# ishine/Prior-DiffuSE

Measured on AMD Instinct MI355X. Metric: enhanced-audio sec/sec (RTF), 6-step fast sampling, B=32, higher is better.
Workload: dtype f16x2; 1 GPU; B=32 x 4 s 16 kHz utterances per GPU, [B,2,401,161] spectrograms, GCRN prior + DiffUNet1 6-step sampling, STFT..ISTFT, seeded random weights; global_batch=32, frames=401, parallelism=batch-shard x1, graph=True, streams_per_gpu=1, batches_in_flight=3

## Files before the change

### include/pdse.h

```cpp
#ifndef PDSE_H
#define PDSE_H
#include <stdint.h>

#ifdef __cplusplus
extern "C" {
#endif

#define PDSE_ABI_VERSION 9

typedef void* pdse_stream_t;

enum pdse_act { PDSE_ACT_NONE = 0, PDSE_ACT_PRELU = 1, PDSE_ACT_ELU = 2, PDSE_ACT_SIGMOID = 3 };

enum pdse_epi {
  PDSE_EPI_LINEAR = 0,
  PDSE_EPI_GLU = 1,
  PDSE_EPI_BIGLU = 2
};

typedef struct pdse_src {
  const float* ptr;
  int64_t sb, sc, st, sf;
  int32_t C;
  int32_t act;
// ... 409 lines not shown
  int64_t bias_sb;
  const float* blc;
  const float* brc;
  const float* bc2;
  float slope;
  int32_t C2;
  float* out;
  int64_t out_sb, out_sc, out_st, out_sf, out_off;
  int32_t hp_par, nx_n;
  uint16_t* nx_hp;
  int64_t nx_hp_sb;
  int32_t nx_Tp, nx_Fp, nx_t0, nx_f0;
  int32_t nx_row0;
  int32_t nx_par;
  const float* nx_add;
  int64_t add_sb, add_sc, add_st, add_sf;
  float* nx_out[2];
  int64_t nx_sb[2], nx_sc[2], nx_st[2], nx_sf[2];
  const float* nx_bias[3];
  int64_t nx_bias_sb[3];
  int32_t skip_Fh;
  int32_t nx_items;
  int32_t qexp[4];
} pdse_bglu_desc;

typedef struct pdse_planes_desc {
  const float* in;
  int64_t in_sb, in_sc, in_st, in_sf;
  uint16_t* hp;
  int64_t hp_sb;
  int32_t hp_Tp, hp_Fp, hp_t0, hp_f0;
  int32_t B, T, F, np;
  const float* in1;
  const float* w[2];
  const float* bias[2];
  int64_t bias_sb;
  uint16_t* hp1;
  int32_t cin0, cin1, nd, pad_;
} pdse_planes_desc;

#define PDSE_METRICS_SSNR 0
#define PDSE_METRICS_LLR 1
#define PDSE_METRICS_WSS 2
#define PDSE_METRICS_FWSNRSEG 3
#define PDSE_METRICS_OFF_WIN 0
#define PDSE_METRICS_OFF_BASIS 512
// ... 157 lines not shown
```

### prior-diffuse_amd/_lib.py

```python
import contextlib
import ctypes as C
import os

_HERE = os.path.dirname(os.path.abspath(__file__))
LIB_PATH = os.environ.get("PDSE_LIB") or os.path.join(_HERE, "libpdse.so")

ABI_VERSION = 9

ACT_NONE, ACT_PRELU, ACT_ELU, ACT_SIGMOID = 0, 1, 2, 3
EPI_LINEAR, EPI_GLU, EPI_BIGLU = 0, 1, 2
EW_DIV, EW_UPDATE, EW_UPDATE_FINAL, EW_COPY, EW_ADD_MUL = 0, 1, 2, 3, 4
(OP_GCONV, OP_TIME, OP_EW, OP_COMPAND, OP_WAVPREP, OP_OLA, OP_SIGMA, OP_LN, OP_LSTM,
 OP_ROWLN, OP_CHLN, OP_ATTN, OP_GRU, OP_GNCOMB, OP_AHAM, OP_QSAMPLE, OP_TRANSPOSE, OP_TCM, OP_CRM, OP_GCRNLAST,
 OP_MASKLOSS, OP_GLSTM, OP_TCM2, OP_BGLU, OP_PLANES, OP_GLSTMP, OP_TCM2S, OP_DENSE, OP_ROWLNB, OP_METRICS, OP_RESAMPLE, OP_RANGE) = range(32)
MASKLOSS_BLOCKS = 32

_fp = C.c_void_p
_i32, _i64, _f32 = C.c_int32, C.c_int64, C.c_float


class Src(C.Structure):
    _fields_ = [("ptr", _fp), ("sb", _i64), ("sc", _i64), ("st", _i64), ("sf", _i64),
                ("C", _i32), ("act", _i32), ("blk", _i32), ("pad_", _i32)]

# ... 155 lines not shown


TCM2S_MAX = 20


class Tcm2sDesc(C.Structure):
    _fields_ = [("blk", Tcm2Desc * TCM2S_MAX), ("flags", _fp), ("status", _fp), ("n", _i32), ("pad_", _i32)]


class BgluDesc(C.Structure):
    _fields_ = [("hp", _fp), ("hp_sb", _i64), ("hp_Tp", _i32), ("hp_Fp", _i32), ("hp_t0", _i32), ("hp_f0", _i32),
                ("x0", Src), ("x1", Src), ("Tin", _i32), ("Fin", _i32), ("ntaps", _i32), ("sf_in", _i32),
                ("tap_dt", _i32 * 10), ("tap_df", _i32 * 10), ("p1mask", _i32), ("Fout1", _i32),
                ("B", _i32), ("Tout", _i32), ("Fout", _i32), ("np", _i32),
                ("w0", _fp), ("w1", _fp), ("w2", _fp), ("w3", _fp), ("wlc", _fp), ("wrc", _fp), ("wc2", _fp), ("wc2v", _fp),
                ("nx_w", _fp), ("bias0", _fp), ("bias1", _fp), ("bias0_t0", _fp), ("bias1_t0", _fp), ("bias_sb", _i64),
                ("blc", _fp), ("brc", _fp), ("bc2", _fp), ("slope", _f32), ("C2", _i32),
                ("out", _fp), ("out_sb", _i64), ("out_sc", _i64), ("out_st", _i64), ("out_sf", _i64), ("out_off", _i64),
                ("hp_par", _i32), ("nx_n", _i32),
                ("nx_hp", _fp), ("nx_hp_sb", _i64), ("nx_Tp", _i32), ("nx_Fp", _i32), ("nx_t0", _i32), ("nx_f0", _i32),
                ("nx_row0", _i32), ("nx_par", _i32),
                ("nx_add", _fp), ("add_sb", _i64), ("add_sc", _i64), ("add_st", _i64), ("add_sf", _i64),
                ("nx_out", _fp * 2), ("nx_sb", _i64 * 2), ("nx_sc", _i64 * 2), ("nx_st", _i64 * 2), ("nx_sf", _i64 * 2),
                ("nx_bias", _fp * 3), ("nx_bias_sb", _i64 * 3), ("skip_Fh", _i32), ("nx_items", _i32), ("qexp", _i32 * 4)]


class PlanesDesc(C.Structure):
    _fields_ = [("in_", _fp), ("in_sb", _i64), ("in_sc", _i64), ("in_st", _i64), ("in_sf", _i64),
                ("hp", _fp), ("hp_sb", _i64), ("hp_Tp", _i32), ("hp_Fp", _i32), ("hp_t0", _i32), ("hp_f0", _i32),
                ("B", _i32), ("T", _i32), ("F", _i32), ("np", _i32),
                ("in1", _fp), ("w", _fp * 2), ("bias", _fp * 2), ("bias_sb", _i64), ("hp1", _fp),
                ("cin0", _i32), ("cin1", _i32), ("nd", _i32), ("pad_", _i32)]


class CrmDesc(C.Structure):
    _fields_ = [("x", _fp), ("o", _fp), ("ri", _fp), ("out", _fp), ("a1", _f32), ("b1", _f32), ("a2", _f32), ("b2", _f32),
                ("a3", _f32), ("b3", _f32), ("plane", _i32), ("B", _i32), ("mode", _i32), ("pad_", _i32)]


class GcrnLastDesc(C.Structure):
    _fields_ = [("in0", _fp), ("in1", _fp), ("w1", _fp), ("w2", _fp), ("fcT", _fp), ("fcb", _fp), ("out", _fp),
                ("out_sb", _i64), ("b1", _f32), ("b2", _f32), ("bn_scale", _f32), ("bn_shift", _f32), ("B", _i32), ("T", _i32),
                ("fcp", _fp)]


class MetricsDesc(C.Structure):
    _fields_ = [("clean", _fp), ("proc", _fp), ("lens_host", _fp), ("lens", _fp), ("tables", _fp), ("frames", _fp),
# ... 238 lines not shown
```

### prior-diffuse_amd/csrc/bglu.hip

```cpp
#include <hip/hip_runtime.h>
#include <stdint.h>
#include <stdio.h>
#include <stdlib.h>

#include "pdse.h"
#include "pdse_internal.h"

#include "gconv_common.h"

#ifndef BGLU_ST_AUX
#define BGLU_ST_AUX 0
#endif

namespace {

#ifdef BGLU_DIAG
__device__ unsigned long long g_bglu_slots[97];
#endif

constexpr int popc(int m) { return m ? (m & 1) + popc(m >> 1) : 0; }
constexpr int rank_of(int m, int tap) { return popc(m & ((1 << tap) - 1)); }

__device__ __forceinline__ void glds16(const void* g, void* l) {
  __builtin_amdgcn_global_load_lds((const __attribute__((address_space(1))) void*)g, (__attribute__((address_space(3))) void*)l,
// ... 92 lines not shown

__device__ __forceinline__ float vmax(const float a, const float b) {
  float r;
  asm("v_max_f32 %0, %1, %2" : "=v"(r) : "v"(a), "v"(b));
  return r;
}

#define BGLU_FLOATS 512
enum { F_BL = 0, F_BR = 32, F_BL0 = 64, F_BR0 = 96, F_BLC = 128, F_BRC = 160, F_BC2 = 192, F_NXB = 256, F_WC2V = 352 };

template <int NT, int P1MASK, int C2, int NXN, bool IN4, int NP>
struct bglu_cfg {
  static constexpr int WV = 8;
  static constexpr int NB = IN4 ? 3 : 2 * NT;
  static constexpr int NT1 = popc(P1MASK), NB1 = 2 * NT1;
  static constexpr bool DUAL = P1MASK != 0;
  static constexpr int BS = NP * 64;
  static constexpr int o_gL = 0, o_gR = NB * BS, o_gL1 = 2 * NB * BS, o_gR1 = o_gL1 + NB1 * BS, o_lc = o_gR1 + NB1 * BS,
                       o_rc = o_lc + 2 * BS, o_c2 = o_rc + 2 * BS, o_nx = o_c2 + (C2 == 64 ? 4 * BS : 0),
                       o_f = o_nx + NXN * 4 * BS;
  static constexpr size_t lds_bytes = (size_t)o_f * sizeof(uint4) + BGLU_FLOATS * sizeof(float);
};

template <int NT, int P1MASK, int C2, int NXN, bool IN4, int NP>
__global__ __launch_bounds__(512, 2) void bglu_kernel(const pdse_bglu_desc d) {
  using CF = bglu_cfg<NT, P1MASK, C2, NXN, IN4, NP>;
  constexpr int WV = CF::WV, NB = CF::NB, NB1 = CF::NB1, BS = CF::BS;
  constexpr bool DUAL = CF::DUAL;
  extern __shared__ uint4 img[];
  const int tid = threadIdx.x;
  const int lane = tid & 63, wave = tid >> 6;
  const int col = lane & 31, h = lane >> 5;
  const int b = blockIdx.y;
  const int P = d.Tout * d.Fout;
  constexpr int PE = NP == 2 ? PDSE_F16_ACT_EXP : 0;
  const int qG = NP == 2 ? d.qexp[0] : 0, qLC = NP == 2 ? d.qexp[1] : 0, qC2 = NP == 2 ? d.qexp[2] : 0, qNX = NP == 2 ? d.qexp[3] : 0;
  [[maybe_unused]] const float s_in = pow2i(PE), s_G = pow2i(-qG), s_LC = pow2i(-(PE + qLC)), s_C2 = pow2i(-qC2), s_NX = pow2i(-qNX),
                               s_C2out = pow2i(-(PE + qC2)), s_NXout = pow2i(-(PE + qNX)), s_NXin = pow2i(PE + qNX);

  {
    const uint4* const srcs[8] = {reinterpret_cast<const uint4*>(d.w0), reinterpret_cast<const uint4*>(d.w1),
                                  reinterpret_cast<const uint4*>(d.w2), reinterpret_cast<const uint4*>(d.w3),
                                  reinterpret_cast<const uint4*>(d.wlc), reinterpret_cast<const uint4*>(d.wrc),
                                  reinterpret_cast<const uint4*>(d.wc2), reinterpret_cast<const uint4*>(d.nx_w)};
    const int cnt[8] = {NB * NP, NB * NP, NB1 * NP, NB1 * NP, 2 * NP, 2 * NP, C2 == 64 ? 4 * NP : 0, NXN * 4 * NP};
    constexpr int total = CF::o_f >> 6;
    for (int c = __builtin_amdgcn_readfirstlane(wave); c < total; c += WV) {
      int cc = c;
// ... 499 lines not shown
      bv[s_][i] = src[(int64_t)(2 * i + h) * d.in_sc];
    }
  };
  request(0, 0);
  for (int k0 = 0; k0 < K; k0 += 64) {
    if (k0 + 32 < K) request(k0 + 32, 1);
#pragma unroll
    for (int i = 0; i < 16; ++i) acc = __builtin_amdgcn_mfma_f32_32x32x2f32(av[0][i], bv[0][i], acc, 0, 0, 0);
    if (k0 + 32 >= K) break;
    if (k0 + 64 < K) request(k0 + 64, 0);
#pragma unroll
    for (int i = 0; i < 16; ++i) acc = __builtin_amdgcn_mfma_f32_32x32x2f32(av[1][i], bv[1][i], acc, 0, 0, 0);
  }
  if (!live) return;
  uint4 p[2][NP];
  split16p<NP>(acc, p, NP == 2 ? pow2i(PDSE_F16_ACT_EXP) : 1.0f);
  uint4* const base = reinterpret_cast<uint4*>((di ? d.hp1 : d.hp) + (int64_t)b * d.hp_sb) + ((int64_t)(t + d.hp_t0) * 4 + h) * (NP * d.hp_Fp) + f + d.hp_f0;
#pragma unroll
  for (int q = 0; q < 2; ++q)
#pragma unroll
    for (int pl = 0; pl < NP; ++pl) base[(2 * q * NP + pl) * d.hp_Fp] = p[q][pl];
}

template <int NT, int P1MASK, int C2, int NXN, bool IN4, int NP>
int launch(const pdse_bglu_desc* d, hipStream_t s) {
  using CF = bglu_cfg<NT, P1MASK, C2, NXN, IN4, NP>;
  const int P = d->Tout * d->Fout;
  const int rounds = (((P + 31) >> 5) + CF::WV - 1) / CF::WV;
  static const int wgs = PDSE_DIAG_ENV("PDSE_BGLU_WGS") ? atoi(PDSE_DIAG_ENV("PDSE_BGLU_WGS")) : 256;
  int gx = (wgs + d->B - 1) / d->B;
  if (gx > rounds) gx = rounds;
  if (gx < 1) gx = 1;
  if (CF::lds_bytes > 160 * 1024) {
    pdse_set_error("bglu: LDS image too large");
    return 1;
  }
  const void* fn = (const void*)bglu_kernel<NT, P1MASK, C2, NXN, IN4, NP>;
  static unsigned long long attr_mask = 0;
  if (pdse_lds_attr(fn, &attr_mask, "bglu lds attribute")) return 1;
#ifdef BGLU_DIAG
  static unsigned long long zs[97];
  for (int k = 0; k < 97; ++k) zs[k] = 0;
  (void)hipMemcpyToSymbol(HIP_SYMBOL(g_bglu_slots), zs, sizeof(zs));
#endif
  hipLaunchKernelGGL((bglu_kernel<NT, P1MASK, C2, NXN, IN4, NP>), dim3(gx, d->B, 1), dim3(64 * CF::WV), CF::lds_bytes, s, *d);
#ifdef BGLU_DIAG
  (void)hipStreamSynchronize(s);
  (void)hipMemcpyFromSymbol(zs, HIP_SYMBOL(g_bglu_slots), sizeof(zs));
  if (zs[96]) {
    fprintf(stderr, "bglu slots NT %d P1 %d C2 %d NXN %d NP %d (cycles per slot and tile, %llu tiles):", NT, P1MASK, C2, NXN, NP, zs[96]);
    double tot = 0;
    for (int k = 0; k < 96; ++k)
      if (zs[k]) {
        fprintf(stderr, " %d:%.0f", k, (double)zs[k] / (double)zs[96]);
        tot += (double)zs[k] / (double)zs[96];
      }
    fprintf(stderr, " | sum %.0f\n", tot);
  }
#endif
  return pdse_check_launch("bglu");
}

template <int NP>
int dispatch(const pdse_bglu_desc* d, hipStream_t s) {
  if (d->x0.ptr) {
    if (d->nx_n == 3) return launch<10, 0, 64, 3, true, NP>(d, s);
  } else if (d->p1mask) {
    if (d->ntaps == 4 && d->p1mask == 5 && d->C2 == 64 && d->nx_n == 1) return launch<4, 5, 64, 1, false, NP>(d, s);
    if (d->ntaps == 6 && d->p1mask == 27 && d->C2 == 1 && d->nx_n == 0) return launch<6, 27, 1, 0, false, NP>(d, s);
  } else {
    if (d->ntaps == 6 && d->C2 == 64 && d->nx_n == 3) return launch<6, 0, 64, 3, false, NP>(d, s);
    if (d->ntaps == 6 && d->C2 == 64 && d->nx_n == 0) return launch<6, 0, 64, 0, false, NP>(d, s);
  }
  pdse_set_error("bglu: no instantiation for this (taps, phases, C2, chained tiles)");
  return 1;
}

}

int pdse_bglu_launch(const pdse_bglu_desc* d, hipStream_t s) {
  if (!d || !d->w0 || !d->w1 || !d->wlc || !d->wrc || !d->bias0 || !d->bias1 || !d->blc || !d->brc || !d->bc2) {
    pdse_set_error("bglu: null operand");
    return 1;
  }
  if (!(d->slope <= 1.0f)) {
    pdse_set_error("bglu: PReLU slope must be <= 1 (max form); use the korder 2 kernels otherwise");
    return 1;
  }
  if (d->B < 1 || d->Tout < 1 || d->Fout < 1 || !(d->np == 3 || d->np == 2 || d->np == 1) || !(d->C2 == 64 || d->C2 == 1) || d->nx_n < 0 ||
      d->nx_n > 3 || d->ntaps < 1 || d->ntaps > 10) {
    pdse_set_error("bglu: bad geometry (np in {1, 2, 3}, C2 in {64, 1}, nx_n <= 3, ntaps <= 10)");
    return 1;
  }
  if (d->p1mask && d->Fout1 > d->Fout) {
    pdse_set_error("bglu: Fout1 > Fout");
    return 1;
  }
  if ((d->C2 == 64 && !d->wc2) || (d->C2 == 1 && (!d->wc2v || !d->out)) || (d->C2 == 64 && d->nx_n == 0 && !d->out) || (d->nx_n > 0 && (!d->nx_w || !d->nx_hp)) ||
      (d->nx_n > 1 && !d->nx_out[0]) || (d->nx_n > 2 && !d->nx_out[1]) || (d->p1mask && (!d->w2 || !d->w3))) {
    pdse_set_error("bglu: an operand of the selected form is missing");
    return 1;
  }
  if (!d->x0.ptr) {
// ... 44 lines not shown
      return ((sb | sc | st | sf) & 3) == 0 && (reinterpret_cast<uintptr_t>(p) & 15) == 0;
    };
    if (d->nx_add && !c4_ok(d->nx_add, d->add_sb, d->add_sc, d->add_st, d->add_sf)) {
      pdse_set_error("bglu: the addend is kept in groups of four channels: strides in multiples of 4 floats, 16-byte aligned base");
      return 1;
    }
    for (int i = 0; i + 1 < d->nx_n; ++i) {
      if ((long long)(d->B + 1) * d->nx_sb[i] * 4 >= (1ll << 32)) {
        pdse_set_error("bglu: skip tensor exceeds 32-bit lane offsets");
        return 1;
      }
      if (!c4_ok(d->nx_out[i], d->nx_sb[i], d->nx_sc[i], d->nx_st[i], d->nx_sf[i])) {
        pdse_set_error("bglu: skip tensors are kept in groups of four channels: strides in multiples of 4 floats, 16-byte aligned base");
        return 1;
      }
    }
  }
  if (d->np == 2) {
    for (int i = 0; i < 4; ++i)
      if (d->qexp[i] < -40 || d->qexp[i] > 40) {
        pdse_set_error("bglu: qexp (f16x2 weight exponents) out of range");
        return 1;
      }
    return dispatch<2>(d, s);
  }
  return d->np == 3 ? dispatch<3>(d, s) : dispatch<1>(d, s);
}

int pdse_bglu_set_form(int form) {
  static int cur = -1;
  if (form < -1 || form > 0) return -2;
  const int prev = cur;
  cur = form;
  return prev;
}

int pdse_planes_launch(const pdse_planes_desc* d, hipStream_t s) {
  if (!d || !d->in || !d->hp || d->B < 1 || d->T < 1 || d->F < 1 || !(d->np == 3 || d->np == 2 || d->np == 1)) {
    pdse_set_error("planes: bad argument");
    return 1;
  }
  if (d->hp_t0 < 0 || d->hp_f0 < 0 || d->hp_t0 + d->T > d->hp_Tp || d->hp_f0 + d->F > d->hp_Fp) {
    pdse_set_error("planes: the tensor does not fit hp");
    return 1;
  }
  if (d->w[0]) {
    if (d->nd < 1 || d->nd > 2 || d->cin0 < 32 || d->cin1 < 0 || (d->cin0 & 31) || (d->cin1 & 31) || d->cin0 + d->cin1 > 128 || (d->cin1 > 0 && !d->in1) || (d->nd == 2 && (!d->w[1] || !d->hp1)) ||
        d->B > 65535) {
      pdse_set_error("planes: the convolution form takes 1 or 2 weight sets, up to 128 input channels (multiples of 32) over one or two sources");
// ... 20 lines not shown
```

### prior-diffuse_amd/csrc/capi.hip

```cpp
#include <hip/hip_runtime.h>
#include <stdint.h>
#include <stdio.h>
#include <string.h>

#include <new>
#include <string>
#include <vector>

#include "pdse.h"
#include "pdse_internal.h"

static thread_local std::string g_err;

void pdse_set_error(const char* msg) { g_err = msg ? msg : "unknown error"; }

int pdse_check_hip(hipError_t e, const char* what) {
  if (e == hipSuccess) return 0;
  g_err = std::string(what) + ": " + hipGetErrorString(e);
  return 1;
}

int pdse_check_launch(const char* what) { return pdse_check_hip(hipGetLastError(), what); }

int pdse_lds_attr(const void* fn, unsigned long long* mask, const char* what) {
// ... 55 lines not shown

static int op_size(int kind) {
  switch (kind) {
#define X(KIND, stem, entry) case PDSE_OP_##KIND: return (int)sizeof(pdse_##stem##_desc);
    PDSE_OPS(X)
#undef X
    default: return -1;
  }
}

static int launch_op(const pdse_op& op, hipStream_t s) {
  switch (op.kind) {
#define X(KIND, stem, entry) case PDSE_OP_##KIND: return pdse_##stem##_launch(&op.d.stem, s);
    PDSE_OPS(X)
#undef X
    default: pdse_set_error("plan: unknown op kind"); return 1;
  }
}

static bool names_odd_phase(const pdse_op& op) {
  return op.kind == PDSE_OP_GCONV && op.d.gconv.korder == 5 && op.d.gconv.p1mask != 0 && op.d.gconv.w2 == nullptr;
}

static int check_follows(const pdse_plan* p, const pdse_op& op) {
  if (p->ops.empty() || !names_odd_phase(p->ops.back())) return 0;
  if (op.kind != PDSE_OP_GCONV) {
    pdse_set_error("plan: the operator behind a gconv that names its odd phase (p1mask, korder 5) must be that phase");
    return 1;
  }
  return pdse_gconv_pair_check(&p->ops.back().d.gconv, &op.d.gconv);
}

static int launch_at(const pdse_plan* p, const int i, const int end, hipStream_t s, int* n) {
  const pdse_op& op = p->ops[i];
  *n = 1;
  if (names_odd_phase(op) && i + 1 < end) {
    *n = 2;
    return pdse_gconv4_pair_launch(&op.d.gconv, &p->ops[i + 1].d.gconv, s);
  }
  return launch_op(op, s);
}

template <typename D>
static int validate_desc(const D*) { return 0; }
static int validate_desc(const pdse_range_desc* d) { return pdse_range_validate(d); }

extern "C" {

int pdse_abi_version(void) { return PDSE_ABI_VERSION; }
const char* pdse_last_error(void) { return g_err.c_str(); }
int pdse_desc_size(int op_kind) { return op_size(op_kind); }

#define X(KIND, stem, entry) \
  int entry(const pdse_##stem##_desc* d, pdse_stream_t s) { return validate_desc(d) ? 1 : pdse_##stem##_launch(d, (hipStream_t)s); }
PDSE_OPS(X)
#undef X

int pdse_plan_create(pdse_plan** out) {
  if (!out) {
    pdse_set_error("plan_create: null out");
    return 1;
// ... 391 lines not shown
```

### prior-diffuse_amd/csrc/pdse_internal.h

```cpp
#ifndef PDSE_INTERNAL_H
#define PDSE_INTERNAL_H
#include <hip/hip_runtime.h>

#include "pdse.h"

void pdse_set_error(const char* msg);
int pdse_check_launch(const char* what);
int pdse_check_hip(hipError_t e, const char* what);
int pdse_lds_attr(const void* fn, unsigned long long* mask, const char* what);
#ifdef PDSE_DIAG
#define PDSE_DIAG_ENV(name) (getenv(name))
#else
#define PDSE_DIAG_ENV(name) ((const char*)nullptr)
#endif

#define PDSE_OPS(X)                                                                            \
  X(GCONV, gconv, pdse_gconv_f32)                                                              \
  X(TIME, time, pdse_time_embed_f32)                                                           \
  X(EW, ew, pdse_ew_f32)                                                                       \
  X(COMPAND, compand, pdse_compand_f32)                                                        \
  X(WAVPREP, wavprep, pdse_wavprep_f32)                                                        \
  X(OLA, ola, pdse_ola_f32)                                                                    \
  X(SIGMA, sigma, pdse_sigma_mask_f32)                                                         \
  X(LN, ln, pdse_layernorm_f32)                                                                \
// ... 11 lines not shown
  X(GCRNLAST, gcrnlast, pdse_gcrnlast_f32)                                                     \
  X(MASKLOSS, maskloss, pdse_masked_mse_f32)                                                   \
  X(GLSTM, glstm, pdse_glstm_f32)                                                              \
  X(TCM2, tcm2, pdse_tcm2_bf16x3)                                                              \
  X(BGLU, bglu, pdse_bglu_planes)                                                              \
  X(PLANES, planes, pdse_split_planes)                                                         \
  X(GLSTMP, glstmp, pdse_glstm_persistent_f32)                             \
  X(TCM2S, tcm2s, pdse_tcm2_stack_bf16x3)    \
  X(DENSE, dense, pdse_dense_layer_bf16x3)                                 \
  X(ROWLNB, rowlnb, pdse_rowln_blocked_f32)                                                    \
  X(METRICS, metrics, pdse_quality_metrics_f32)                          \
  X(RESAMPLE, resample, pdse_pcm_resample_f32)                          \
  X(RANGE, range, pdse_range_hist)

#define X(KIND, stem, entry) int pdse_##stem##_launch(const pdse_##stem##_desc* d, hipStream_t s);
PDSE_OPS(X)
#undef X
int pdse_gconv2_launch(const pdse_gconv_desc* d, hipStream_t s);
int pdse_gconv3_launch(const pdse_gconv_desc* d, hipStream_t s);
int pdse_gconv4_launch(const pdse_gconv_desc* d, hipStream_t s);
int pdse_gconv_pair_check(const pdse_gconv_desc* d, const pdse_gconv_desc* e);
int pdse_gconv4_pair_check(const pdse_gconv_desc* d, const pdse_gconv_desc* e);
int pdse_gconv4_pair_launch(const pdse_gconv_desc* d, const pdse_gconv_desc* e, hipStream_t s);
int pdse_stoi_launch(const pdse_metrics_desc* d, hipStream_t s);
int pdse_gru3_launch(const pdse_gru_desc* d, hipStream_t s);
int pdse_range_validate(const pdse_range_desc* d);
#endif
```

### prior-diffuse_amd/nets.py

```python
import ctypes as C

import numpy as np
import torch

from . import _lib as L
from . import packing as P

F0 = 161
BIG = 1 << 30

TAG_NONE, TAG_EPS_BLOCK, TAG_EPS_CONV1, TAG_TCM, TAG_PRIOR, TAG_LSTM, TAG_SIGNAL, TAG_EW = range(8)


class WeightBank:

    def __init__(self):
        self.items = {}
        self.keep = []
        self.owners = []

    def token(self, obj):
        if obj is None:
            return None
        for i, o in enumerate(self.owners):
# ... 226 lines not shown


def nc8(C_, T, F):
    return C_ * T * F, T * F * 8, F * 8, 8


def nc8_out(C_, T, F):
    return C_ * T * F, T * F * 8, 1, F * 8, 8


class EpsNetPlan(PlanBase):

    ENC_F = [161, 79, 39, 19, 9, 4]
    fused_tcm = True
    chain_conv1 = True
    compose_stage1 = True
    split_bf16 = True
    split_tcm = True
    plane_h = True
    tcm_stack = True
    parity_planes = True
    planes = 2
    TCM_F16 = True
    NSLOT = 20

    def __init__(self, ctx, sd, B, T, time_cond=True, nsteps=1, plan=None, table=None, with_pre=None, split_bf16=None,
                 planes=None, plane_h=None, exclusive=False, frames=None):
        with_pre = time_cond if with_pre is None else with_pre
        if split_bf16 is not None:
            self.split_bf16 = bool(split_bf16)
        if planes is not None:
            if int(planes) not in (1, 2, 3):
                raise ValueError("planes is 3 (bf16x3), 2 (f16x2) or 1 (bf16 mode)")
            self.planes = int(planes)
        if plane_h is not None:
            self.plane_h = bool(plane_h)
        if self.planes == 1:
            self.plane_h = True
        self.tcm_planes = 3 if (self.planes == 2 and not self.TCM_F16) else self.planes
        self.use_tcm_stack = bool(self.tcm_stack and exclusive)
        self.frames = frames
        if frames is not None and (self.force_generic or not self.fused_tcm):
            raise ValueError("exact ragged batches need a fused TCM form (csrc/tcm.hip, csrc/tcm2.hip): the three-launch form has no frames table")
        self.sd = sd
        ok = (self.split_bf16 and self.chain_conv1 and self.compose_stage1 and time_cond and with_pre and not self.force_generic
              and all(float(P._np(sd[k])[0]) <= 1.0 for k in sd if k.endswith(".weight") and P._np(sd[k]).shape == (1,)))
        if not ok:
            if self.planes == 1:
                raise ValueError("bf16 mode needs the chained split-bf16 DiffUNet1 path (PReLU slopes <= 1)")
            self.plane_h = False
            if self.planes == 2:
                self.planes = self.tcm_planes = 3
        super().__init__(ctx, plan, ns=(ctx.bank.token(sd), bool(time_cond), bool(with_pre), self.fused_tcm, self.chain_conv1,
                                        self.compose_stage1, self.split_bf16, self.split_tcm,
                                        ctx.bank.token(table), str(self.plane_h), self.planes, self.parity_planes))
        self.sd, self.B, self.T, self.time_cond, self.nsteps = sd, B, T, time_cond, nsteps
        self.with_pre = with_pre
        a = ctx.alloc
        self.x = a(B, 2, T, F0)
        self.x_init = a(B, 2, T, F0) if self.with_pre else None
        self.out = a(B, 2, T, F0)
        self.H = a(B, 32, T + 1, F0)
        self.H2 = a(B, 32, T + 1, F0)
        self.Pskip = [[None] + [a(B + 1, 32, T, self.ENC_F[k]) for k in range(1, 5)] for _ in range(2)]
        self.zero32 = self.upw("zero32", lambda: np.zeros(32))
        self.en = [a(B, 64, T, f) for f in self.ENC_F[1:5]] + [a(B, 64, 4, T)]
        self.tcm_a, self.tcm_b = a(B, 256, T), a(B, 256, T)
        self.tcm_h, self.tcm_g = a(B, 64, T), a(B, 64, T)
        self.tcm_hs = [ctx.alloc_u16(*P.tcm2_hs_shape(B, T, self.tcm_planes)) for _ in range(2)]
        self._tcm_stack = None
        self.tcm_flags = torch.zeros(B * ((T + 31) // 32), dtype=torch.int32, device=ctx.device)
        self.tcm_status = torch.zeros(4, dtype=torch.int32, device=ctx.device)
        ctx.keep += [self.tcm_flags, self.tcm_status]
        self.dec = [a(B, 64, T, 79), a(B, 64, T, 79)]
        if self.plane_h:
            self.hp_en = {k: ctx.alloc_u16(*P.hp_shape(B + 1, T, self.ENC_F[k - 1], self.planes)) for k in range(2, 6)}
            self.hp_de = {k: ctx.alloc_u16(*P.hp_shape(B + 1, T, self.ENC_F[k], self.planes)) for k in range(1, 6)}
            self.hp_de5b = ctx.alloc_u16(*P.hp_shape(B + 1, T, self.ENC_F[5], self.planes))
            for k, t_ in self.hp_en.items():
                self.named("hp_en%d" % k, t_)
            for k, t_ in self.hp_de.items():
                self.named("hp_de%d" % k, t_)
            self.named("hp_de5b", self.hp_de5b)
        for name, t_ in (("x", self.x), ("x_init", self.x_init), ("en5", self.en[4]), ("tcm_a", self.tcm_a), ("tcm_b", self.tcm_b),
                         ("tcm_hs0", self.tcm_hs[0]), ("tcm_hs1", self.tcm_hs[1])):
            if t_ is not None:
                self.named(name, t_)
        if time_cond:
            self.tsteps = a(nsteps, B, zero=True)
            self.tbias = a(nsteps, B, self.NSLOT * 32)
            self.temb = a(nsteps, B, 512)
            self._prep_time(table)

    def w(self, k):
        return P._np(self.sd[k])

    def _stage_fold(self):
        st = []
        for k in range(1, 6):
            W1 = self.w("en.conv%d.conv1.weight" % k)[:, :, 0, 0]
# ... 240 lines not shown

    def _residual_split(self, p, dil, xin, xout, hin, hout, p_next, mode=0):
        npl = self.tcm_planes
        d = L.Tcm2Desc()
        self.apply(d, self.fields("%s.split%d.np%d" % (p if mode == 0 else p_next, mode, npl),
                                  lambda: P.tcm2_fields(self.sd, p, p_next, npl, mode)))
        d.x = xin.data_ptr()
        if mode == 0:
            d.x_out, d.hs = xout.data_ptr(), hin.data_ptr()
        if p_next is not None:
            d.hs_out = hout.data_ptr()
        d.dil, d.B, d.T, d.mode, d.np = dil, self.B, self.T, mode, npl
        d.frames = Ctx.ptr(self.frames)
        if mode == 0 and self._tcm_stack is not None:
            self._tcm_stack.append(d)
        else:
            self.add(d, TAG_TCM)

    def _plane_stage(self, kind):
        return self.plane_h is True

    def _bglu(self, label, make, *, hp=None, F_in=None, x0=None, x1=None, taps, sf_in, Fout, p1mask=0, Fout1=0, slope, C2,
              bias, out=None, out_strides=None, out_off=0, nx_hp=None, nx_F=None, nx_row0=False, nx_add=None,
              nx_out=(), nx_bias=(), hp_par=False, nx_par=False, skip_F=0):
        B, T, npl = self.B, self.T, self.planes
        d = L.BgluDesc()
        self.apply(d, self.fields("bglu:%s:%d" % (label, npl), make))
        if hp is not None:
            shp = P.hp_shape(B + 1, T, F_in, npl)
            d.hp, d.hp_sb, d.hp_Tp, d.hp_Fp, d.hp_t0, d.hp_f0 = hp.data_ptr(), int(np.prod(shp[1:])), shp[1], shp[4], P.HP_T0, P.HP_F0
            d.hp_par = 1 if hp_par else 0
        else:
            d.x0, d.x1 = x0, x1
        d.Tin, d.Fin = T, (F_in if F_in is not None else F0)
        d.ntaps, d.sf_in = len(taps), sf_in
        for i, (dt_, df_) in enumerate(taps):
            d.tap_dt[i], d.tap_df[i] = int(dt_), int(df_)
        d.p1mask, d.Fout1 = p1mask, Fout1
        d.B, d.Tout, d.Fout, d.np = B, T, Fout, npl
        tb, o0, o1, o0t, o1t, sb = bias
        if tb is not None:
            d.bias0, d.bias1, d.bias_sb = Ctx.ptr(tb, o0), Ctx.ptr(tb, o1), sb
            if o0t is not None:
                d.bias0_t0, d.bias1_t0 = Ctx.ptr(tb, o0t), Ctx.ptr(tb, o1t)
        d.slope, d.C2 = float(slope), C2
        if out is not None:
            d.out = Ctx.ptr(out)
            d.out_sb, d.out_sc, d.out_st, d.out_sf = out_strides
            d.out_off = out_off
        d.skip_Fh = (skip_F + 1) // 2 if (skip_F and self.parity_planes) else 0
        d.nx_n = (1 if nx_hp is not None else 0) + len(nx_out)
        d.nx_items = B + 1
        assert all(t_.shape[0] == B + 1 for t_, *_ in nx_out) and (nx_hp is None or nx_hp.shape[0] == B + 1)
        if nx_hp is not None:
            shp = P.hp_shape(B + 1, T, nx_F, npl)
            d.nx_hp, d.nx_hp_sb, d.nx_Tp, d.nx_Fp, d.nx_t0, d.nx_f0 = (nx_hp.data_ptr(), int(np.prod(shp[1:])), shp[1], shp[4],
                                                                      P.HP_T0, P.HP_F0)
            d.nx_row0 = 1 if nx_row0 else 0
            d.nx_par = 1 if nx_par else 0
        if nx_add is not None:
            t_, sb_, sc_, st_, sf_ = nx_add
            d.nx_add, d.add_sb, d.add_sc, d.add_st, d.add_sf = Ctx.ptr(t_), sb_, sc_, st_, sf_
        for i, (t_, sb_, sc_, st_, sf_) in enumerate(nx_out):
            d.nx_out[i] = Ctx.ptr(t_)
            d.nx_sb[i], d.nx_sc[i], d.nx_st[i], d.nx_sf[i] = sb_, sc_, st_, sf_
        for i, (t_, off_, sb_) in enumerate(nx_bias):
            d.nx_bias[i], d.nx_bias_sb[i] = Ctx.ptr(t_, off_), sb_
        self.add(d, TAG_EPS_BLOCK)
        return d

    def _encoder_planes(self, step, x, x_init):
        B, T, npl = self.B, self.T, self.planes
        sbb = self.NSLOT * 32
        tb = self.tbias

        def slot(sl):
            return self._bias_for(step, sl)[1]

        for k in range(1, 6):
            p = "en.conv%d" % k
            Fin, Fo = self.ENC_F[k - 1], self.ENC_F[k]
            kw = 5 if k == 1 else 3
            kk, taps = P.conv_taps(2, kw, 1)
            chained = k < 5
            pn = "en.conv%d" % (k + 1)

            def nx_weights(k=k, pn=pn):
                if k == 5:
                    return []
                ws = [self.w(pn + ".conv1.weight")[:, :, 0, 0]]
# ... 16 lines not shown
            kwargs = dict(taps=taps, sf_in=2, Fout=Fo, slope=self._slope("en.en%d.1.weight" % k), C2=64, **src)
            if chained:
                sk = [(self.Pskip[di][k], 32 * T * Fo, 4 * T * Fo, 4 * Fo, 4) for di in range(2)]
                kwargs.update(nx_hp=self.hp_en[k + 1], nx_F=Fo, nx_row0=True, nx_out=sk, nx_par=self.parity_planes, skip_F=Fo,
                              nx_bias=[(tb, slot(k), sbb)] + [(tb, slot(5 + 5 * di + (5 - k)), sbb) for di in range(2)])
            else:
                kwargs.update(out=self.en[4], out_strides=(64 * 4 * T, 4 * T, 1, T))
            self._bglu("en%d" % k, make, bias=bias or (None, 0, 0, None, None, 0), **kwargs)

    def _decoders_planes(self, step, tcm_out, out):
        B, T, npl = self.B, self.T, self.planes
        pd = L.PlanesDesc()
        pd.in_, pd.in1 = tcm_out.data_ptr(), self.en[4].data_ptr()
        pd.in_sb, pd.in_sc, pd.in_st, pd.in_sf = 256 * T, 4 * T, 1, T
        shp = P.hp_shape(B + 1, T, 4, npl)
        pd.hp, pd.hp1 = self.hp_de[5].data_ptr(), self.hp_de5b.data_ptr()
        pd.hp_sb, pd.hp_Tp, pd.hp_Fp, pd.hp_t0, pd.hp_f0 = int(np.prod(shp[1:])), shp[1], shp[4], P.HP_T0, P.HP_F0
        pd.B, pd.T, pd.F, pd.np, pd.cin0, pd.cin1, pd.nd = B, T, 4, npl, 64, 64, 2
        for di, de in enumerate(("de_real", "de_imag")):
            tb, off, sbb = self._bias_for(step, 5 + 5 * di)
            pd.w[di] = self.upw("%s.de5.0.conv1.kmajor" % de, lambda de=de: self.w("%s.de5.0.conv1.weight" % de)[:, :, 0, 0]).data_ptr()
            pd.bias[di], pd.bias_sb = Ctx.ptr(tb, off), sbb
        self.add(pd, TAG_EPS_CONV1)
        for di, de in enumerate(("de_real", "de_imag")):
            for n, k in enumerate((5, 4, 3, 2, 1)):
                p = "%s.de%d.0" % (de, k)
                Fin = self.ENC_F[k]
                kw = 5 if k == 1 else 3
                Fo = 2 * (Fin - 1) + kw
                kk0, taps0 = P.convT_phase_taps(2, kw, 0)
                kk1, taps1 = P.convT_phase_taps(2, kw, 1)
                mask = sum(1 << taps0.index(tp) for tp in taps1)
                C2 = 64 if k > 1 else 1
                bn = "%s.de%d.2" % (de, k) if k > 1 else None

                def make(p=p, k=k, de=de, kk0=kk0, kk1=kk1, C2=C2, bn=bn):
                    g = dict(w0=P.convT_kmat(self.sd[p + ".l.weight"], kk0), w1=P.convT_kmat(self.sd[p + ".r.weight"], kk0),
                             w2=P.convT_kmat(self.sd[p + ".l.weight"], kk1), w3=P.convT_kmat(self.sd[p + ".r.weight"], kk1))
                    nxw = [self.w("%s.de%d.0.conv1.weight" % (de, k - 1))[:, :, 0, 0].T[:, :64]] if k > 1 else []
                    return P.bglu_fields(self.sd, p, True, C2, bn, g, nxw, npl, True)

                kwargs = dict(hp=self.hp_de5b if (k == 5 and di == 1) else self.hp_de[k], F_in=Fin, taps=taps0, sf_in=1, Fout=(Fo + 1) // 2, p1mask=mask, Fout1=Fo // 2,
                              slope=self._slope("%s.de%d.3.weight" % (de, k)) if k > 1 else 1.0, C2=C2,
                              bias=(None, 0, 0, None, None, 0))
                if k > 1:
                    kwargs.update(nx_hp=self.hp_de[k - 1], nx_F=Fo, nx_add=(self.Pskip[di][k - 1], 32 * T * Fo, 4 * T * Fo, 4 * Fo, 4), skip_F=Fo,
                                  nx_bias=[(self.zero32, 0, 0)])
                else:
                    kwargs.update(out=out, out_strides=(2 * T * F0, T * F0, F0, 2), out_off=di * T * F0)
                self._bglu(p, make, **kwargs)

    def build_step(self, step=0, x=None, x_init=None, out=None):
        B, T = self.B, self.T
        x = self.x if x is None else x
        out = self.out if out is None else out
        x_init = self.x_init if x_init is None else x_init
        key = (x.data_ptr(), 0 if x_init is None else x_init.data_ptr(), out.data_ptr())
        tmpl = getattr(self, "_tmpl", None)
        if tmpl is not None and tmpl[0] == key and self.time_cond:
            _, step0, items = tmpl
            lo = self.tbias.data_ptr()
            hi = lo + self.tbias.numel() * 4
            delta = (step - step0) * B * self.NSLOT * 32 * 4
            for d, tag in items:
                d2 = type(d).from_buffer_copy(d)
                if isinstance(d2, L.GconvDesc):
                    for f in ("bias0", "bias1", "bias0_t0", "bias1_t0", "padrow"):
                        v = getattr(d2, f)
                        if v and lo <= v < hi:
                            setattr(d2, f, v + delta)
                    for i in range(d2.nx_n):
                        v = d2.nx_bias[i]
                        if v and lo <= v < hi:
# ... 806 lines not shown
```

Baseline: 10010 audio_s/s.

## Pair real and imaginary decoder BGLU blocks into one launch per stage

Reorders the decoder so each stage's real and imaginary BGLU blocks sit next to each other, and runs the two twins as a single kernel launch. blockIdx.z selects which twin's descriptor a block uses. The decoder plane buffers are doubled so each twin gets its own slice, and a validation step checks the twins share geometry and do not overlap in memory. This removes five launches per step and fills the GPU with twice as many workgroups for the small decoder stages, at the cost of a larger kernel argument block and more plane memory.

```diff
diff --git a/include/pdse.h b/include/pdse.h
--- a/include/pdse.h
+++ b/include/pdse.h
@@ -455,6 +455,7 @@
   int32_t skip_Fh;
   int32_t nx_items;
   int32_t qexp[4];
+  int32_t pair, pad_;
 } pdse_bglu_desc;
 
 typedef struct pdse_planes_desc {
diff --git a/prior-diffuse_amd/_lib.py b/prior-diffuse_amd/_lib.py
--- a/prior-diffuse_amd/_lib.py
+++ b/prior-diffuse_amd/_lib.py
@@ -201,7 +201,8 @@
                 ("nx_row0", _i32), ("nx_par", _i32),
                 ("nx_add", _fp), ("add_sb", _i64), ("add_sc", _i64), ("add_st", _i64), ("add_sf", _i64),
                 ("nx_out", _fp * 2), ("nx_sb", _i64 * 2), ("nx_sc", _i64 * 2), ("nx_st", _i64 * 2), ("nx_sf", _i64 * 2),
-                ("nx_bias", _fp * 3), ("nx_bias_sb", _i64 * 3), ("skip_Fh", _i32), ("nx_items", _i32), ("qexp", _i32 * 4)]
+                ("nx_bias", _fp * 3), ("nx_bias_sb", _i64 * 3), ("skip_Fh", _i32), ("nx_items", _i32), ("qexp", _i32 * 4),
+                ("pair", _i32), ("pad_", _i32)]
 
 
 class PlanesDesc(C.Structure):
diff --git a/prior-diffuse_amd/csrc/bglu.hip b/prior-diffuse_amd/csrc/bglu.hip
--- a/prior-diffuse_amd/csrc/bglu.hip
+++ b/prior-diffuse_amd/csrc/bglu.hip
@@ -138,8 +138,17 @@
   static constexpr size_t lds_bytes = (size_t)o_f * sizeof(uint4) + BGLU_FLOATS * sizeof(float);
 };
 
-template <int NT, int P1MASK, int C2, int NXN, bool IN4, int NP>
-__global__ __launch_bounds__(512, 2) void bglu_kernel(const pdse_bglu_desc d) {
+struct alignas(64) bglu_slot {
+  pdse_bglu_desc d;
+};
+template <bool PAIR>
+struct bglu_args {
+  bglu_slot s[PAIR ? 2 : 1];
+};
+
+template <int NT, int P1MASK, int C2, int NXN, bool IN4, int NP, bool PAIR>
+__global__ __launch_bounds__(512, 2) void bglu_kernel(const bglu_args<PAIR> args) {
+  const pdse_bglu_desc& d = args.s[PAIR ? blockIdx.z : 0].d;
   using CF = bglu_cfg<NT, P1MASK, C2, NXN, IN4, NP>;
   constexpr int WV = CF::WV, NB = CF::NB, NB1 = CF::NB1, BS = CF::BS;
   constexpr bool DUAL = CF::DUAL;
@@ -685,20 +694,21 @@
     for (int pl = 0; pl < NP; ++pl) base[(2 * q * NP + pl) * d.hp_Fp] = p[q][pl];
 }
 
-template <int NT, int P1MASK, int C2, int NXN, bool IN4, int NP>
-int launch(const pdse_bglu_desc* d, hipStream_t s) {
+template <int NT, int P1MASK, int C2, int NXN, bool IN4, int NP, bool PAIR = false>
+int launch(const pdse_bglu_desc* d, hipStream_t s, const pdse_bglu_desc* e = nullptr) {
   using CF = bglu_cfg<NT, P1MASK, C2, NXN, IN4, NP>;
   const int P = d->Tout * d->Fout;
   const int rounds = (((P + 31) >> 5) + CF::WV - 1) / CF::WV;
   static const int wgs = PDSE_DIAG_ENV("PDSE_BGLU_WGS") ? atoi(PDSE_DIAG_ENV("PDSE_BGLU_WGS")) : 256;
-  int gx = (wgs + d->B - 1) / d->B;
+  const int items = PAIR ? 2 * d->B : d->B;
+  int gx = (wgs + items - 1) / items;
   if (gx > rounds) gx = rounds;
   if (gx < 1) gx = 1;
   if (CF::lds_bytes > 160 * 1024) {
     pdse_set_error("bglu: LDS image too large");
     return 1;
   }
-  const void* fn = (const void*)bglu_kernel<NT, P1MASK, C2, NXN, IN4, NP>;
+  const void* fn = (const void*)bglu_kernel<NT, P1MASK, C2, NXN, IN4, NP, PAIR>;
   static unsigned long long attr_mask = 0;
   if (pdse_lds_attr(fn, &attr_mask, "bglu lds attribute")) return 1;
 #ifdef BGLU_DIAG
@@ -706,7 +716,10 @@
   for (int k = 0; k < 97; ++k) zs[k] = 0;
   (void)hipMemcpyToSymbol(HIP_SYMBOL(g_bglu_slots), zs, sizeof(zs));
 #endif
-  hipLaunchKernelGGL((bglu_kernel<NT, P1MASK, C2, NXN, IN4, NP>), dim3(gx, d->B, 1), dim3(64 * CF::WV), CF::lds_bytes, s, *d);
+  bglu_args<PAIR> args;
+  args.s[0].d = *d;
+  if constexpr (PAIR) args.s[1].d = *e;
+  hipLaunchKernelGGL((bglu_kernel<NT, P1MASK, C2, NXN, IN4, NP, PAIR>), dim3(gx, d->B, PAIR ? 2 : 1), dim3(64 * CF::WV), CF::lds_bytes, s, args);
 #ifdef BGLU_DIAG
   (void)hipStreamSynchronize(s);
   (void)hipMemcpyFromSymbol(zs, HIP_SYMBOL(g_bglu_slots), sizeof(zs));
@@ -725,6 +738,14 @@
 }
 
 template <int NP>
+int dispatch_pair(const pdse_bglu_desc* d, const pdse_bglu_desc* e, hipStream_t s) {
+  if (d->ntaps == 4 && d->p1mask == 5 && d->C2 == 64 && d->nx_n == 1) return launch<4, 5, 64, 1, false, NP, true>(d, s, e);
+  if (d->ntaps == 6 && d->p1mask == 27 && d->C2 == 1 && d->nx_n == 0) return launch<6, 27, 1, 0, false, NP, true>(d, s, e);
+  pdse_set_error("bglu: no paired instantiation for this (taps, phases, C2, chained tiles)");
+  return 1;
+}
+
+template <int NP>
 int dispatch(const pdse_bglu_desc* d, hipStream_t s) {
   if (d->x0.ptr) {
     if (d->nx_n == 3) return launch<10, 0, 64, 3, true, NP>(d, s);
@@ -741,7 +762,7 @@
 
 }
 
-int pdse_bglu_launch(const pdse_bglu_desc* d, hipStream_t s) {
+static int bglu_validate(const pdse_bglu_desc* d) {
   if (!d || !d->w0 || !d->w1 || !d->wlc || !d->wrc || !d->bias0 || !d->bias1 || !d->blc || !d->brc || !d->bc2) {
     pdse_set_error("bglu: null operand");
     return 1;
@@ -832,9 +853,63 @@
         pdse_set_error("bglu: qexp (f16x2 weight exponents) out of range");
         return 1;
       }
-    return dispatch<2>(d, s);
-  }
-  return d->np == 3 ? dispatch<3>(d, s) : dispatch<1>(d, s);
+  }
+  if (d->pair < 0 || d->pair > 1 || (d->pair && d->x0.ptr)) {
+    pdse_set_error("bglu: pair is 0 or 1 (the next operator is this block's twin), on plane input only");
+    return 1;
+  }
+  return 0;
+}
+
+int pdse_bglu_launch(const pdse_bglu_desc* d, hipStream_t s) {
+  if (bglu_validate(d)) return 1;
+  return d->np == 2 ? dispatch<2>(d, s) : d->np == 3 ? dispatch<3>(d, s) : dispatch<1>(d, s);
+}
+
+int pdse_bglu_pair_check(const pdse_bglu_desc* d, const pdse_bglu_desc* e) {
+  if (bglu_validate(d) || bglu_validate(e)) return 1;
+  if (!d->pair || e->pair || d->x0.ptr || e->x0.ptr) {
+    pdse_set_error("bglu pair: the first block names its twin (pair 1), the twin names none; plane input only");
+    return 1;
+  }
+  bool same = d->np == e->np && d->ntaps == e->ntaps && d->sf_in == e->sf_in && d->p1mask == e->p1mask && d->Fout1 == e->Fout1 && d->B == e->B &&
+              d->Tout == e->Tout && d->Fout == e->Fout && d->C2 == e->C2 && d->nx_n == e->nx_n && d->Tin == e->Tin && d->Fin == e->Fin &&
+              d->hp_sb == e->hp_sb && d->hp_Tp == e->hp_Tp && d->hp_Fp == e->hp_Fp && d->hp_t0 == e->hp_t0 && d->hp_f0 == e->hp_f0 && d->hp_par == e->hp_par &&
+              d->nx_hp_sb == e->nx_hp_sb && d->nx_Tp == e->nx_Tp && d->nx_Fp == e->nx_Fp && d->nx_t0 == e->nx_t0 && d->nx_f0 == e->nx_f0 &&
+              d->nx_row0 == e->nx_row0 && d->nx_par == e->nx_par && d->skip_Fh == e->skip_Fh && d->nx_items == e->nx_items &&
+              d->add_sb == e->add_sb && d->add_sc == e->add_sc && d->add_st == e->add_st && d->add_sf == e->add_sf &&
+              d->out_sb == e->out_sb && d->out_sc == e->out_sc && d->out_st == e->out_st && d->out_sf == e->out_sf;
+  for (int i = 0; i < d->ntaps && same; ++i) same = d->tap_dt[i] == e->tap_dt[i] && d->tap_df[i] == e->tap_df[i];
+  for (int i = 0; i + 1 < d->nx_n && same; ++i)
+    same = d->nx_sb[i] == e->nx_sb[i] && d->nx_sc[i] == e->nx_sc[i] && d->nx_st[i] == e->nx_st[i] && d->nx_sf[i] == e->nx_sf[i];
+  if (!same) {
+    pdse_set_error("bglu pair: the twins differ in geometry (planes, taps, phases, extents, strides or layout flags)");
+    return 1;
+  }
+  auto overlap = [](const void* a, const long long na, const void* b, const long long nb) {
+    const uintptr_t a0 = reinterpret_cast<uintptr_t>(a), b0 = reinterpret_cast<uintptr_t>(b);
+    return a && b && a0 < b0 + (uintptr_t)nb && b0 < a0 + (uintptr_t)na;
+  };
+  const long long in_b = (long long)d->B * d->hp_sb * 2, nx_b = d->nx_n > 0 ? (long long)(d->B + 1) * d->nx_hp_sb * 2 : 0;
+  bool clash = false;
+  if (d->nx_n > 0)
+    clash = overlap(d->nx_hp, nx_b, e->nx_hp, nx_b) || overlap(d->nx_hp, nx_b, e->hp, in_b) || overlap(e->nx_hp, nx_b, d->hp, in_b) ||
+            overlap(d->nx_hp, nx_b, d->hp, in_b) || overlap(e->nx_hp, nx_b, e->hp, in_b);
+  for (int i = 0; i + 1 < d->nx_n && !clash; ++i) {
+    const long long sk_b = (long long)(d->B + 1) * d->nx_sb[i] * 4;
+    for (int k = 0; k + 1 < d->nx_n && !clash; ++k) clash = overlap(d->nx_out[i], sk_b, e->nx_out[k], (long long)(d->B + 1) * d->nx_sb[k] * 4);
+  }
+  if (d->out && (d->C2 == 1 || d->nx_n == 0)) clash = clash || d->out + d->out_off == e->out + e->out_off;
+  if (clash) {
+    pdse_set_error("bglu pair: an output of one twin overlaps an operand of the other");
+    return 1;
+  }
+  return 0;
+}
+
+int pdse_bglu_pair_launch(const pdse_bglu_desc* d, const pdse_bglu_desc* e, hipStream_t s) {
+  if (pdse_bglu_pair_check(d, e)) return 1;
+  return d->np == 2 ? dispatch_pair<2>(d, e, s) : d->np == 3 ? dispatch_pair<3>(d, e, s) : dispatch_pair<1>(d, e, s);
 }
 
 int pdse_bglu_set_form(int form) {
diff --git a/prior-diffuse_amd/csrc/capi.hip b/prior-diffuse_amd/csrc/capi.hip
--- a/prior-diffuse_amd/csrc/capi.hip
+++ b/prior-diffuse_amd/csrc/capi.hip
@@ -101,7 +101,16 @@
   return op.kind == PDSE_OP_GCONV && op.d.gconv.korder == 5 && op.d.gconv.p1mask != 0 && op.d.gconv.w2 == nullptr;
 }
 
+static bool names_twin(const pdse_op& op) { return op.kind == PDSE_OP_BGLU && op.d.bglu.pair != 0; }
+
 static int check_follows(const pdse_plan* p, const pdse_op& op) {
+  if (!p->ops.empty() && names_twin(p->ops.back())) {
+    if (op.kind != PDSE_OP_BGLU) {
+      pdse_set_error("plan: the operator behind a bglu block that names its twin (pair) must be that twin");
+      return 1;
+    }
+    return pdse_bglu_pair_check(&p->ops.back().d.bglu, &op.d.bglu);
+  }
   if (p->ops.empty() || !names_odd_phase(p->ops.back())) return 0;
   if (op.kind != PDSE_OP_GCONV) {
     pdse_set_error("plan: the operator behind a gconv that names its odd phase (p1mask, korder 5) must be that phase");
@@ -116,6 +125,10 @@
   if (names_odd_phase(op) && i + 1 < end) {
     *n = 2;
     return pdse_gconv4_pair_launch(&op.d.gconv, &p->ops[i + 1].d.gconv, s);
+  }
+  if (names_twin(op) && i + 1 < end) {
+    *n = 2;
+    return pdse_bglu_pair_launch(&op.d.bglu, &p->ops[i + 1].d.bglu, s);
   }
   return launch_op(op, s);
 }
diff --git a/prior-diffuse_amd/csrc/pdse_internal.h b/prior-diffuse_amd/csrc/pdse_internal.h
--- a/prior-diffuse_amd/csrc/pdse_internal.h
+++ b/prior-diffuse_amd/csrc/pdse_internal.h
@@ -57,6 +57,8 @@
 int pdse_gconv_pair_check(const pdse_gconv_desc* d, const pdse_gconv_desc* e);
 int pdse_gconv4_pair_check(const pdse_gconv_desc* d, const pdse_gconv_desc* e);
 int pdse_gconv4_pair_launch(const pdse_gconv_desc* d, const pdse_gconv_desc* e, hipStream_t s);
+int pdse_bglu_pair_check(const pdse_bglu_desc* d, const pdse_bglu_desc* e);
+int pdse_bglu_pair_launch(const pdse_bglu_desc* d, const pdse_bglu_desc* e, hipStream_t s);
 int pdse_stoi_launch(const pdse_metrics_desc* d, hipStream_t s);
 int pdse_gru3_launch(const pdse_gru_desc* d, hipStream_t s);
 int pdse_range_validate(const pdse_range_desc* d);
diff --git a/prior-diffuse_amd/nets.py b/prior-diffuse_amd/nets.py
--- a/prior-diffuse_amd/nets.py
+++ b/prior-diffuse_amd/nets.py
@@ -272,6 +272,8 @@
     parity_planes = True
     planes = 2
     TCM_F16 = True
+    pair_decoders = True
+    pair_stages = (5, 4, 3, 2, 1)
     NSLOT = 20
 
     def __init__(self, ctx, sd, B, T, time_cond=True, nsteps=1, plan=None, table=None, with_pre=None, split_bf16=None,
@@ -303,7 +305,8 @@
                 self.planes = self.tcm_planes = 3
         super().__init__(ctx, plan, ns=(ctx.bank.token(sd), bool(time_cond), bool(with_pre), self.fused_tcm, self.chain_conv1,
                                         self.compose_stage1, self.split_bf16, self.split_tcm,
-                                        ctx.bank.token(table), str(self.plane_h), self.planes, self.parity_planes))
+                                        ctx.bank.token(table), str(self.plane_h), self.planes, self.parity_planes,
+                                        bool(self.pair_decoders)))
         self.sd, self.B, self.T, self.time_cond, self.nsteps = sd, B, T, time_cond, nsteps
         self.with_pre = with_pre
         a = ctx.alloc
@@ -325,7 +328,7 @@
         self.dec = [a(B, 64, T, 79), a(B, 64, T, 79)]
         if self.plane_h:
             self.hp_en = {k: ctx.alloc_u16(*P.hp_shape(B + 1, T, self.ENC_F[k - 1], self.planes)) for k in range(2, 6)}
-            self.hp_de = {k: ctx.alloc_u16(*P.hp_shape(B + 1, T, self.ENC_F[k], self.planes)) for k in range(1, 6)}
+            self.hp_de = {k: ctx.alloc_u16(*P.hp_shape((B + 1) * (1 if k == 5 else 2), T, self.ENC_F[k], self.planes)) for k in range(1, 6)}
             self.hp_de5b = ctx.alloc_u16(*P.hp_shape(B + 1, T, self.ENC_F[5], self.planes))
             for k, t_ in self.hp_en.items():
                 self.named("hp_en%d" % k, t_)
@@ -612,7 +615,7 @@
 
     def _bglu(self, label, make, *, hp=None, F_in=None, x0=None, x1=None, taps, sf_in, Fout, p1mask=0, Fout1=0, slope, C2,
               bias, out=None, out_strides=None, out_off=0, nx_hp=None, nx_F=None, nx_row0=False, nx_add=None,
-              nx_out=(), nx_bias=(), hp_par=False, nx_par=False, skip_F=0):
+              nx_out=(), nx_bias=(), hp_par=False, nx_par=False, skip_F=0, pair=False):
         B, T, npl = self.B, self.T, self.planes
         d = L.BgluDesc()
         self.apply(d, self.fields("bglu:%s:%d" % (label, npl), make))
@@ -656,6 +659,7 @@
             d.nx_sb[i], d.nx_sc[i], d.nx_st[i], d.nx_sf[i] = sb_, sc_, st_, sf_
         for i, (t_, off_, sb_) in enumerate(nx_bias):
             d.nx_bias[i], d.nx_bias_sb[i] = Ctx.ptr(t_, off_), sb_
+        d.pair = 1 if pair else 0
         self.add(d, TAG_EPS_BLOCK)
         return d
 
@@ -718,33 +722,41 @@
             pd.w[di] = self.upw("%s.de5.0.conv1.kmajor" % de, lambda de=de: self.w("%s.de5.0.conv1.weight" % de)[:, :, 0, 0]).data_ptr()
             pd.bias[di], pd.bias_sb = Ctx.ptr(tb, off), sbb
         self.add(pd, TAG_EPS_CONV1)
-        for di, de in enumerate(("de_real", "de_imag")):
-            for n, k in enumerate((5, 4, 3, 2, 1)):
-                p = "%s.de%d.0" % (de, k)
-                Fin = self.ENC_F[k]
-                kw = 5 if k == 1 else 3
-                Fo = 2 * (Fin - 1) + kw
-                kk0, taps0 = P.convT_phase_taps(2, kw, 0)
-                kk1, taps1 = P.convT_phase_taps(2, kw, 1)
-                mask = sum(1 << taps0.index(tp) for tp in taps1)
-                C2 = 64 if k > 1 else 1
-                bn = "%s.de%d.2" % (de, k) if k > 1 else None
-
-                def make(p=p, k=k, de=de, kk0=kk0, kk1=kk1, C2=C2, bn=bn):
-                    g = dict(w0=P.convT_kmat(self.sd[p + ".l.weight"], kk0), w1=P.convT_kmat(self.sd[p + ".r.weight"], kk0),
-                             w2=P.convT_kmat(self.sd[p + ".l.weight"], kk1), w3=P.convT_kmat(self.sd[p + ".r.weight"], kk1))
-                    nxw = [self.w("%s.de%d.0.conv1.weight" % (de, k - 1))[:, :, 0, 0].T[:, :64]] if k > 1 else []
-                    return P.bglu_fields(self.sd, p, True, C2, bn, g, nxw, npl, True)
-
-                kwargs = dict(hp=self.hp_de5b if (k == 5 and di == 1) else self.hp_de[k], F_in=Fin, taps=taps0, sf_in=1, Fout=(Fo + 1) // 2, p1mask=mask, Fout1=Fo // 2,
-                              slope=self._slope("%s.de%d.3.weight" % (de, k)) if k > 1 else 1.0, C2=C2,
-                              bias=(None, 0, 0, None, None, 0))
-                if k > 1:
-                    kwargs.update(nx_hp=self.hp_de[k - 1], nx_F=Fo, nx_add=(self.Pskip[di][k - 1], 32 * T * Fo, 4 * T * Fo, 4 * Fo, 4), skip_F=Fo,
-                                  nx_bias=[(self.zero32, 0, 0)])
-                else:
-                    kwargs.update(out=out, out_strides=(2 * T * F0, T * F0, F0, 2), out_off=di * T * F0)
-                self._bglu(p, make, **kwargs)
+
+        def hp_of(k, di):
+            if k == 5:
+                return self.hp_de5b if di == 1 else self.hp_de[5]
+            return self.hp_de[k][di * (B + 1):(di + 1) * (B + 1)]
+
+        pair = bool(self.pair_decoders)
+        order = [(k, di) for k in (5, 4, 3, 2, 1) for di in range(2)] if pair else [(k, di) for di in range(2) for k in (5, 4, 3, 2, 1)]
+        for k, di in order:
+            de = ("de_real", "de_imag")[di]
+            p = "%s.de%d.0" % (de, k)
+            Fin = self.ENC_F[k]
+            kw = 5 if k == 1 else 3
+            Fo = 2 * (Fin - 1) + kw
+            kk0, taps0 = P.convT_phase_taps(2, kw, 0)
+            kk1, taps1 = P.convT_phase_taps(2, kw, 1)
+            mask = sum(1 << taps0.index(tp) for tp in taps1)
+            C2 = 64 if k > 1 else 1
+            bn = "%s.de%d.2" % (de, k) if k > 1 else None
+
+            def make(p=p, k=k, de=de, kk0=kk0, kk1=kk1, C2=C2, bn=bn):
+                g = dict(w0=P.convT_kmat(self.sd[p + ".l.weight"], kk0), w1=P.convT_kmat(self.sd[p + ".r.weight"], kk0),
+                         w2=P.convT_kmat(self.sd[p + ".l.weight"], kk1), w3=P.convT_kmat(self.sd[p + ".r.weight"], kk1))
+                nxw = [self.w("%s.de%d.0.conv1.weight" % (de, k - 1))[:, :, 0, 0].T[:, :64]] if k > 1 else []
+                return P.bglu_fields(self.sd, p, True, C2, bn, g, nxw, npl, True)
+
+            kwargs = dict(hp=hp_of(k, di), F_in=Fin, pair=pair and di == 0 and k in self.pair_stages, taps=taps0, sf_in=1, Fout=(Fo + 1) // 2, p1mask=mask, Fout1=Fo // 2,
+                          slope=self._slope("%s.de%d.3.weight" % (de, k)) if k > 1 else 1.0, C2=C2,
+                          bias=(None, 0, 0, None, None, 0))
+            if k > 1:
+                kwargs.update(nx_hp=hp_of(k - 1, di), nx_F=Fo, nx_add=(self.Pskip[di][k - 1], 32 * T * Fo, 4 * T * Fo, 4 * Fo, 4), skip_F=Fo,
+                              nx_bias=[(self.zero32, 0, 0)])
+            else:
+                kwargs.update(out=out, out_strides=(2 * T * F0, T * F0, F0, 2), out_off=di * T * F0)
+            self._bglu(p, make, **kwargs)
 
     def build_step(self, step=0, x=None, x_init=None, out=None):
         B, T = self.B, self.T
```

Result: no change. 10070 audio_s/s, median of 6 (+0.6%).
